# praateekmahajan/moving-mnist-vae

Hardware: AMD Instinct MI355X
Metric: frames/sec/GPU VAE train step, 20×64×64 batch; ELBO vs CPU ref (higher is better)
Workload: dtype bf16; 1 GPU; BASELINE configs[1]: 256 clips x 20 frames x 64x64 per GPU per step (=5120 frames), conv-VAE z=128, Gaussian NLL sigma=0.1 + KL (normal_vae_1_kl_0_mmd), Adam, random-init weights, Bernoulli(0.0521) q=2 labels; parallelism=dp1, rccl_ranks=1, grad_exchange=none, bn=per-rank batch statistics

## Files before the change

### include/mmvae.h

```cpp
#ifndef MMVAE_H_
#define MMVAE_H_

#include <stddef.h>
#include <stdint.h>

#ifdef __cplusplus
extern "C" {
#endif

#if defined(__GNUC__)
#define MMVAE_API __attribute__((visibility("default")))
#else
#define MMVAE_API
#endif

#define MMVAE_OK 0
#define MMVAE_ERR_ARG (-1)
#define MMVAE_ERR_HIP (-2)
#define MMVAE_ERR_WORKSPACE (-3)
#define MMVAE_ERR_UNSUPPORTED (-4)

#define MMVAE_F32 0
#define MMVAE_BF16 1
#define MMVAE_FP8 2
// ... 189 lines not shown
                               const float* b2, const void* ys, const float* ss, const float* bs, float* partials, float* wpartials,
                               int N, int H, int W, void* stream);
MMVAE_API int mmvae_tail_join_bwd_apply(int dtype, const float* d_raw, const float* weight, int out_planes, const void* y2, const float* s2,
                              const float* b2, const void* ys, const float* ss, const float* bs, const float* A2, const float* B2,
                              const float* C2, const float* As, const float* Bs, const float* Cs, void* dy2, void* dys, int N, int H, int W,
                              void* stream);
MMVAE_API int mmvae_upblock_bwd_fused(const float* d_raw, const float* tail_weight, const void* y2, const float* s2, const float* b2,
                            const void* ys, const float* ss, const float* bs, const float* A2, const float* B2, const float* C2,
                            const float* As, const float* Bs, const float* Cs, const void* y1, const float* s1, const float* b1,
                            const float* w_conv2, float* dw_conv2, void* d_a1, float* bn1_sums, const void* xin, const float* sx,
                            const float* bx, const float* w_up, float* dw_up, void* g_in, int N, void* scratch, void* stream);
MMVAE_API int mmvae_upblock_tail_fwd(const void* y1, const float* s1, const float* b1, const float* w2, const void* x_in, const float* sx,
                                     const float* bx, const float* wu, const float* s2, const float* b2, const float* ss, const float* bs,
                                     const float* tail_weight, const float* tail_bias, float* r_raw, float* stats, int N, void* scratch,
                                     void* stream);
MMVAE_API int mmvae_join_conv1x1_fwd(const void* y2, const float* s2, const float* b2, const void* ys, const float* ss, const float* bs,
                           const float* w_conv1, int C, void* out, void* y1, float* stats, int64_t npix, void* scratch, void* stream);
MMVAE_API int mmvae_conv1x1_bwd_fused(const void* d_a1, const void* y1, const float* s1, const float* b1, const float* A1, const float* B1,
                            const float* C1, const void* xin, const float* sx, const float* bx, const float* w_conv1, float* dw_conv1,
                            void* g_in, int64_t rows, void* scratch, void* stream);
typedef struct mmvae_pixelcnn mmvae_pixelcnn;
MMVAE_API int mmvae_pixelcnn_create(mmvae_pixelcnn** out, int in_channels, int intermediate_channels, int out_channels, int layers, int dtype);
MMVAE_API void mmvae_pixelcnn_destroy(mmvae_pixelcnn* net);
MMVAE_API int64_t mmvae_pixelcnn_num_params(mmvae_pixelcnn* net);
MMVAE_API size_t mmvae_pixelcnn_workspace_bytes(mmvae_pixelcnn* net, int N, int S);
MMVAE_API int mmvae_pixelcnn_fwd(mmvae_pixelcnn* net, int N, int S, const float* x, const float* params, void* workspace, size_t workspace_bytes,
                       float* out, void* stream);
MMVAE_API int mmvae_pixelcnn_bwd(mmvae_pixelcnn* net, int N, int S, const float* x, const float* d_out, const float* params, float* grads,
                       void* workspace, size_t workspace_bytes, float* d_x, void* stream);
MMVAE_API size_t mmvae_pixelcnn_sample_workspace_bytes(mmvae_pixelcnn* net, int N, int S);
// ... 11 lines not shown
```

### moving-mnist-vae_amd/_lib.py

```python
from __future__ import annotations

import ctypes
import os
from ctypes import POINTER, c_char_p, c_double, c_float, c_int, c_int32, c_int64, c_size_t, c_uint64, c_void_p

import torch

_HERE = os.path.dirname(os.path.abspath(__file__))
LIB_PATH = os.environ.get("MMVAE_LIB_PATH") or os.path.join(_HERE, "libmmvae_hip.so")
_lib = None
ABI_VERSION = 3
SUM_PARTIALS = 1025
BN_SCRATCH_BYTES = 16 << 20
STEM_SCRATCH_BYTES = 12800

P = c_void_p

PROTOTYPES = {
    "mmvae_abi_version": (c_int, []),
    "mmvae_last_error": (c_char_p, []),
    "mmvae_net_create": (c_int, [POINTER(c_void_p), c_int, c_int, c_int, c_int, c_int, c_int]),
    "mmvae_net_create_ex": (c_int, [POINTER(c_void_p), c_int, c_int, c_int, c_int, c_int, c_int, c_int]),
    "mmvae_net_destroy": (None, [P]),
    "mmvae_net_sizes": (c_int, [P, POINTER(c_int64), POINTER(c_int64), POINTER(c_int32), POINTER(c_int64), POINTER(c_int32)]),
# ... 68 lines not shown
    "mmvae_net_set_sync_bn_comm": (c_int, [P, P]),
    "mmvae_net_set_sync_bn_comm2": (c_int, [P, P, P]),
    "mmvae_convT_bwd_fused": (c_int, [c_int, P, P, P, P, P, c_int, c_int, c_int, c_int, c_int, c_int, c_int, c_int, P, P, c_int, P, P, P, P, P, P]),
    "mmvae_batchnorm_fwd": (c_int, [c_int, P, c_int64, c_int, P, P, P, P, P, c_float, c_float, c_int, P, P, P, P, P]),
    "mmvae_batchnorm_bwd": (c_int, [c_int, P, P, P, c_int64, c_int, P, P, P, P, P, P, P, P]),
    "mmvae_stem_fwd": (c_int, [c_int, P, P, P, c_int, c_int, P, P, P]),
    "mmvae_stem_bwd": (c_int, [c_int, P, P, P, P, P, P, P, P, P, P, P, P, c_int, c_int, P, P]),
    "mmvae_tail_join_fwd": (c_int, [c_int, P, P, P, P, P, P, P, P, P, P, c_int, c_int, c_int, P]),
    "mmvae_tail_join_fwd_stream": (c_int, [c_int, P, P, P, P, P, P, P, P, P, P, c_int, c_int, c_int, P]),
    "mmvae_tail_join_bwd_reduce": (c_int, [c_int, P, P, c_int, P, P, P, P, P, P, P, P, c_int, c_int, c_int, P]),
    "mmvae_tail_join_bwd_apply": (c_int, [c_int, P, P, c_int, P, P, P, P, P, P, P, P, P, P, P, P, P, P, c_int, c_int, c_int, P]),
    "mmvae_upblock_bwd_fused": (c_int, [P] * 27 + [c_int, P, P]),
    "mmvae_join_conv1x1_fwd": (c_int, [P, P, P, P, P, P, P, c_int, P, P, P, c_int64, P, P]),
    "mmvae_conv1x1_bwd_fused": (c_int, [P] * 13 + [c_int64, P, P]),
    "mmvae_upblock_tail_fwd": (c_int, [P] * 16 + [c_int, P, P]),
    "mmvae_pixelcnn_create": (c_int, [POINTER(c_void_p), c_int, c_int, c_int, c_int, c_int]),
    "mmvae_pixelcnn_destroy": (None, [P]),
    "mmvae_pixelcnn_num_params": (c_int64, [P]),
    "mmvae_pixelcnn_workspace_bytes": (c_size_t, [P, c_int, c_int]),
    "mmvae_pixelcnn_fwd": (c_int, [P, c_int, c_int, P, P, P, c_size_t, P, P]),
    "mmvae_pixelcnn_bwd": (c_int, [P, c_int, c_int, P, P, P, P, P, c_size_t, P, P]),
    "mmvae_pixelcnn_sample_workspace_bytes": (c_size_t, [P, c_int, c_int]),
    "mmvae_pixelcnn_sample": (c_int, [P, c_int, c_int, P, c_int, P, c_int, P, c_float, c_float, P, P, c_size_t, P, P, P, P]),
    "mmvae_convert": (c_int, [c_int, c_int, P, P, c_int64, P]),
}


class MmvaeError(RuntimeError):
    pass

# ... 71 lines not shown
```

### moving-mnist-vae_amd/csrc/capi.cpp

```cpp
#include <cstring>
#include <new>

#include "../../include/mmvae.h"
#include "conv_ops.hpp"
#include "pixel_net.hpp"
#include "quantiser_fit.hpp"
#include "resample.hpp"
#include "vae_net.hpp"

namespace mmvae { const char* last_error(); }
using namespace mmvae;

struct mmvae_net { Net* net; };
struct mmvae_comm { Comm* c; };

static inline hipStream_t stream_of(void* s) { return static_cast<hipStream_t>(s); }

extern "C" {

int mmvae_abi_version(void) { return MMVAE_ABI_VERSION; }
const char* mmvae_last_error(void) { return last_error(); }

int mmvae_net_create(mmvae_net** out, int in_channels, int z, int out_channels, int image_size, int need_logvar, int dtype) {
  return mmvae_net_create_ex(out, in_channels, z, out_channels, image_size, need_logvar, dtype, 1);
// ... 592 lines not shown
  }
  return launch_partial_rowsum(L.bn_part, nb, 32, bn1_sums, stream_of(st));
}
int mmvae_upblock_tail_fwd(const void* y1, const float* s1, const float* b1, const float* w2, const void* xin, const float* sx, const float* bx,
                           const float* wu, const float* s2, const float* b2, const float* ss, const float* bs, const float* tw, const float* bias,
                           float* r_raw, float* stats, int N, void* scratch, void* st) {
  if (!scratch || !y1 || !s1 || !b1 || !w2 || !xin || !wu || !s2 || !b2 || !ss || !bs || !tw || !r_raw || N < 1 || ((sx != nullptr) != (bx != nullptr))) {
    set_error("upblock_tail_fwd: bad argument"); return MMVAE_ERR_ARG;
  }
  char* sc = static_cast<char*>(scratch);
  const ConvGeom g = geom_for(1, 16, 16, 4, 2, 1);
  int rc = op_pack_up(DT_BF16, g, w2, sc, stream_of(st)); if (rc < 0) return rc;
  rc = op_pack_up(DT_BF16, g, wu, sc + 8192, stream_of(st)); if (rc < 0) return rc;
  return launch_up5_tail_fwd(y1, s1, b1, sc, xin, sx, bx, sc + 8192, s2, b2, ss, bs, tw, bias, r_raw, stats, N, stream_of(st));
}
int mmvae_conv1x1_bwd_fused(const void* da1, const void* y1, const float* s1, const float* b1, const float* A1, const float* B1, const float* C1,
                            const void* xin, const float* sx, const float* bx, const float* w1, float* dw1, void* gin, int64_t rows, void* scratch,
                            void* st) {
  if (!scratch || !da1 || !y1 || !s1 || !b1 || !A1 || !B1 || !C1 || !xin || !w1 || !dw1 || !gin || rows < 1 || ((sx != nullptr) != (bx != nullptr))) {
    set_error("conv1x1_bwd_fused: bad argument"); return MMVAE_ERR_ARG;
  }
  char* sc = static_cast<char*>(scratch);
  const ConvGeom g = geom_for(0, 16, 16, 1, 1, 0);
  int rc = op_pack_up(DT_BF16, g, w1, sc, stream_of(st)); if (rc < 0) return rc;
  Conv1BwdLaunch C;
  C.da1 = da1; C.y1 = y1; C.ms = s1; C.mb = b1; C.A = A1; C.B = B1; C.C = C1; C.xin = xin; C.pxs = sx; C.pxb = bx; C.w1u = sc; C.gin = gin;
  C.part = reinterpret_cast<float*>(sc + 4096); C.nrows = (long)rows;
  const int nb = launch_conv1_bwd_stream(C, stream_of(st));
  if (nb < 0) return nb;
  WgradReduceArgs u; std::memset(&u, 0, sizeof(u));
// ... 15 lines not shown
```

### moving-mnist-vae_amd/csrc/conv_fstream.hip

```cpp
#include <hip/hip_runtime.h>

#include <stdlib.h>
#include <string.h>

#include "kernels.hpp"
#include "tile_common.hpp"

namespace mmvae {

struct Conv3StreamArgs {
  const void* x; const void* w; const void* wsc; void* y; void* ysc;
  const float* pro_scale; const float* pro_shift; int pro_relu;
  float* stats; float* stats_sc;
  const void* ym; const float* ms; const float* mb;
  int N, Ho, Hi;
  int HS, nunits;
};

template <int S, bool SC, bool PRO, bool BS = false>
__global__ __launch_bounds__(256, 2) void conv3_stream_kernel(Conv3StreamArgs a) {
  static_assert(!BS || (S == 1 && !SC && !PRO), "backward sums: the stride-1 data gradient");
  constexpr int KS = 3, PAD = 1, WO = 16, WI = S * WO, CB = 64;
  constexpr int WL = WI + 2;
  constexpr int ROWB = WL * CB;
// ... 331 lines not shown
  }
  st1 = row16_sum(st1); st2 = row16_sum(st2);
  float* sb = reinterpret_cast<float*>(smem);
  if (lane == 0) { sb[wv * 2] = st1; sb[wv * 2 + 1] = st2; }
  __syncthreads();
  if (a.stats && t < 2) a.stats[(long)blockIdx.x * 2 + t] = (sb[t] + sb[2 + t]) + (sb[4 + t] + sb[6 + t]);
}

struct ConvT4StreamArgs {
  const void* x; const void* w; void* y;
  const float* pro_scale; const float* pro_shift; int pro_relu;
  float* stats;
  int N, Hi, HS, nunits;
};

template <int WIN, bool PRO, bool F8O = false>
__global__ __launch_bounds__(256, 3) void convT4_stream_kernel(ConvT4StreamArgs a) {
  constexpr int CB = 32, WL = WIN + 2, ROWB = WL * CB, NSLOT = 4, NPRIME = 2;
  constexpr int CBO = F8O ? 16 : 32;
  constexpr int OROWB = 2 * WIN * CBO;
  constexpr int WAVE_LDS = NSLOT * ROWB + OROWB;
  constexpr int XV = (WIN * CB + 1023) / 1024;
  constexpr int NPT = WIN / 16;
  extern __shared__ __attribute__((aligned(16))) char smem[];
  const int t = threadIdx.x, lane = t & 63, wv = __builtin_amdgcn_readfirstlane(t >> 6), gq = lane >> 4, r = lane & 15;
  char* ring = smem + 1024 + wv * WAVE_LDS;
  char* orow = ring + NSLOT * ROWB;
  for (int s = 0; s < NSLOT; ++s) {
    if (lane < 2) *reinterpret_cast<Vec16*>(ring + s * ROWB + lane * 16) = Vec16{{0, 0, 0, 0}};
    else if (lane < 4) *reinterpret_cast<Vec16*>(ring + s * ROWB + (WL - 1) * CB + (lane - 2) * 16) = Vec16{{0, 0, 0, 0}};
  }
  Vec16 wA[4][2];
#pragma unroll
  for (int p = 0; p < 4; ++p)
#pragma unroll
    for (int th = 0; th < 2; ++th)
// ... 26 lines not shown
  };
  auto commit = [&](int u, int q) {
    const int n = u / nstrips, q0 = (u - n * nstrips) * a.HS;
    const int row = q0 + q - NPRIME + 1;
    if (xlane) {
      Vec16 v = xv;
      if (PRO && row >= 0 && row < a.Hi) {
        float f[8];
        Elem<bf16_t>::unpack(v, f);
#pragma unroll
        for (int j = 0; j < 8; ++j) f[j] = fmaxf(f[j] * psc[j] + psh[j], lo);
        v = Elem<bf16_t>::pack(f);
      }
      *reinterpret_cast<Vec16*>(ring + ((row + 4 * NSLOT) % NSLOT) * ROWB + CB + lane * 16) = v;
    }
    (void)n; (void)XV;
  };
  int u = u_first, q = 0;
  if (u < u_end) issue(u, 0);
  while (u < u_end) {
    commit(u, q);
    int un = u, qn = q + 1;
    if (qn == nq) { un = u + u_step; qn = 0; }
    if (un < u_end) issue(un, qn);
    __builtin_amdgcn_sched_barrier(0);
    if (q >= NPRIME) {
      const int n = u / nstrips, iq = (u - n * nstrips) * a.HS + q - NPRIME;
#pragma unroll
      for (int ph = 0; ph < 2; ++ph) {
#pragma unroll
        for (int pw = 0; pw < 2; ++pw) {
// ... 2 lines not shown
          for (int pt = 0; pt < NPT; ++pt) acc[pt] = (f32x4){0, 0, 0, 0};
#pragma unroll
          for (int th = 0; th < 2; ++th) {
            const int dh = ph == 0 ? (th == 0 ? 0 : -1) : (th == 0 ? 1 : 0);
            const char* rowp = ring + ((iq + dh + 4 * NSLOT) % NSLOT) * ROWB;
#pragma unroll
            for (int pt = 0; pt < NPT; ++pt) {
              const Vec16 b = *reinterpret_cast<const Vec16*>(rowp + (16 * pt + r + dwl[pw] + 1) * CB + (gq & 1) * 16);
              acc[pt] = mma_bf16(wA[2 * ph + pw][th], b, acc[pt]);
            }
          }
#pragma unroll
          for (int pt = 0; pt < NPT; ++pt) {
#pragma unroll
            for (int j = 0; j < 4; ++j) { st1[j] += acc[pt][j]; st2[j] += acc[pt][j] * acc[pt][j]; }
            if constexpr (F8O) {
              *reinterpret_cast<uint32_t*>(orow + (2 * (16 * pt + r) + pw) * CBO + gq * 4) = pack4_fp8(acc[pt][0], acc[pt][1], acc[pt][2], acc[pt][3]);
            } else {
              uint2 o;
              o.x = pack2_bf16(acc[pt][0], acc[pt][1]); o.y = pack2_bf16(acc[pt][2], acc[pt][3]);
              *reinterpret_cast<uint2*>(orow + (2 * (16 * pt + r) + pw) * CB + gq * 8) = o;
            }
          }
        }
        asm volatile("" ::: "memory");
        char* dst = reinterpret_cast<char*>(a.y) + (((long)n * (2 * a.Hi) + 2 * iq + ph) * (2 * WIN)) * CBO;
#pragma unroll
        for (int k = 0; k < OROWB / 1024; ++k) *reinterpret_cast<Vec16*>(dst + (lane + 64 * k) * 16) = *reinterpret_cast<const Vec16*>(orow + (lane + 64 * k) * 16);
      }
    }
    __builtin_amdgcn_sched_barrier(0);
    u = un; q = qn;
  }
  float* sb = reinterpret_cast<float*>(smem);
#pragma unroll
  for (int j = 0; j < 4; ++j) {
    const float v1 = row16_sum(st1[j]), v2 = row16_sum(st2[j]);
    if (r == 0) { sb[wv * 32 + 4 * gq + j] = v1; sb[wv * 32 + 16 + 4 * gq + j] = v2; }
  }
  __syncthreads();
  if (a.stats && t < 32) a.stats[(long)blockIdx.x * 32 + t] = (sb[t] + sb[32 + t]) + (sb[64 + t] + sb[96 + t]);
}

struct Up5TailFwdArgs {
  const void* y1; const float* p1s; const float* p1b; const void* w2;
  const void* xin; const float* pxs; const float* pxb; const void* wu;
  const float* s2; const float* b2; const float* ss; const float* bs;
  const float* w; const float* bias; float* r_raw; float* stats;
  int N, HS, nunits;
};

template <bool PRO_X>
__global__ __launch_bounds__(256, 2) void up5_tail_fwd_kernel(Up5TailFwdArgs a) {
  constexpr int WIN = 32, Hi = 32, W = 64, H = 64, CB = 32;
  constexpr int IWL = WIN + 2, IROWB = IWL * CB, NSLOT = 4;
  constexpr int JWL = W + 2, JROWB = JWL * CB;
  constexpr int WAVE_LDS = 2 * NSLOT * IROWB + NSLOT * JROWB;
  extern __shared__ __attribute__((aligned(16))) char smem[];
  const int t = threadIdx.x, lane = t & 63, wv = __builtin_amdgcn_readfirstlane(t >> 6), gq = lane >> 4, r = lane & 15;
  char* ringA = smem + 64 + wv * WAVE_LDS;
  char* ringX = ringA + NSLOT * IROWB;
  char* ringJ = ringX + NSLOT * IROWB;
  for (int sl = 0; sl < NSLOT; ++sl) {
    if (lane < 2) { *reinterpret_cast<Vec16*>(ringA + sl * IROWB + lane * 16) = Vec16{{0, 0, 0, 0}}; *reinterpret_cast<Vec16*>(ringX + sl * IROWB + lane * 16) = Vec16{{0, 0, 0, 0}}; }
    else if (lane < 4) { *reinterpret_cast<Vec16*>(ringA + sl * IROWB + (IWL - 1) * CB + (lane - 2) * 16) = Vec16{{0, 0, 0, 0}}; *reinterpret_cast<Vec16*>(ringX + sl * IROWB + (IWL - 1) * CB + (lane - 2) * 16) = Vec16{{0, 0, 0, 0}}; }
    else if (lane < 6) *reinterpret_cast<Vec16*>(ringJ + sl * JROWB + (lane - 4) * 16) = Vec16{{0, 0, 0, 0}};
    else if (lane < 8) *reinterpret_cast<Vec16*>(ringJ + sl * JROWB + (JWL - 1) * CB + (lane - 6) * 16) = Vec16{{0, 0, 0, 0}};
// ... 72 lines not shown
    *reinterpret_cast<Vec16*>(ringX + slot * IROWB + CB + lane * 16) = cx;
    (void)n;
  };
  int u = u_first, q = 0;
  if (u < u_end) issue(u, 0);
  while (u < u_end) {
    commit(u, q);
    int un = u, qn = q + 1;
    if (qn == nq) { un = u + u_step; qn = 0; }
    if (un < u_end) issue(un, qn);
    __builtin_amdgcn_sched_barrier(0);
    if (q >= NPRIME) {
      const int n = u / nstrips, q0 = (u - n * nstrips) * a.HS;
      const int iq = q0 - 1 + q - NPRIME;
      const bool inside = iq >= 0 && iq < Hi;
#pragma unroll
      for (int ph = 0; ph < 2; ++ph) {
        char* jrow = ringJ + ((2 * iq + ph + 8 * NSLOT) % NSLOT) * JROWB;
        if (!inside) {
          for (int i = lane; i < (W * CB) / 16; i += 64) *reinterpret_cast<Vec16*>(jrow + CB + i * 16) = Vec16{{0, 0, 0, 0}};
          continue;
        }
#pragma unroll
        for (int pw = 0; pw < 2; ++pw) {
          f32x4 acc2[2], accS[2];
#pragma unroll
          for (int pt = 0; pt < 2; ++pt) { acc2[pt] = (f32x4){0, 0, 0, 0}; accS[pt] = (f32x4){0, 0, 0, 0}; }
#pragma unroll
          for (int th = 0; th < 2; ++th) {
            const int dh = ph == 0 ? (th == 0 ? 0 : -1) : (th == 0 ? 1 : 0);
            const int sl = (iq + dh + 4 * NSLOT) % NSLOT;
#pragma unroll
            for (int pt = 0; pt < 2; ++pt) {
              const int off = sl * IROWB + (16 * pt + r + dwl[pw] + 1) * CB + (gq & 1) * 16;
              acc2[pt] = mma_bf16(w2A[2 * ph + pw][th], *reinterpret_cast<const Vec16*>(ringA + off), acc2[pt]);
              accS[pt] = mma_bf16(wuA[2 * ph + pw][th], *reinterpret_cast<const Vec16*>(ringX + off), accS[pt]);
            }
          }
#pragma unroll
          for (int pt = 0; pt < 2; ++pt) {
            float o[4];
#pragma unroll
            for (int j = 0; j < 4; ++j) o[j] = fmaxf(acc2[pt][j] * js2[j] + jb[j] + accS[pt][j] * jss[j], 0.f);
            *reinterpret_cast<uint2*>(jrow + (1 + 2 * (16 * pt + r) + pw) * CB + gq * 8) = make_uint2(pack2_bf16(o[0], o[1]), pack2_bf16(o[2], o[3]));
          }
        }
      }
      asm volatile("" ::: "memory");
#pragma unroll
      for (int k = 0; k < 2; ++k) {
        const int oh = 2 * iq - 1 + k;
        if (oh < 2 * q0 || oh >= 2 * (q0 + a.HS) || oh < 0 || oh >= H) continue;
        f32x4 acc[4];
        const char* row01 = ringJ + ((oh - 1 + (gq >> 1) + 8 * NSLOT) % NSLOT) * JROWB;
        const char* row2 = ringJ + ((oh + 1 + 8 * NSLOT) % NSLOT) * JROWB;
#pragma unroll
        for (int pt = 0; pt < 4; ++pt) {
          const int po = (16 * pt + r + 1) * CB + (gq & 1) * 16;
          acc[pt] = mma_bf16(wT[0], *reinterpret_cast<const Vec16*>(row01 + po), (f32x4){0, 0, 0, 0});
// ... 33 lines not shown
    __builtin_amdgcn_sched_barrier(0);
    u = un; q = qn;
  }
  st1 = row16_sum(st1); st2 = row16_sum(st2);
  float* sb = reinterpret_cast<float*>(smem);
  if (lane == 0) { sb[wv * 2] = st1; sb[wv * 2 + 1] = st2; }
  __syncthreads();
  if (a.stats && t < 2) a.stats[(long)blockIdx.x * 2 + t] = (sb[t] + sb[2 + t]) + (sb[4 + t] + sb[6 + t]);
}

bool up5_tail_fwd_ok(int dt, int OC, int C, int Cin, int Hin, int Hout) {
  return dt == DT_BF16 && OC == 1 && C == 16 && Cin == 16 && Hin == 32 && Hout == 64;
}
int launch_up5_tail_fwd(const void* y1, const float* p1s, const float* p1b, const void* w2_up, const void* xin, const float* pxs, const float* pxb,
                        const void* wu_up, const float* s2, const float* b2, const float* ss, const float* bs, const float* w, const float* bias,
                        float* r_raw, float* stats, int N, hipStream_t s) {
  Up5TailFwdArgs a; memset(&a, 0, sizeof(a));
  a.y1 = y1; a.p1s = p1s; a.p1b = p1b; a.w2 = w2_up; a.xin = xin; a.pxs = pxs; a.pxb = pxb; a.wu = wu_up;
  a.s2 = s2; a.b2 = b2; a.ss = ss; a.bs = bs; a.w = w; a.bias = bias; a.r_raw = r_raw; a.stats = stats;
  a.N = N; a.HS = 16; a.nunits = N * (32 / a.HS);
  int gx = 512;
  while (gx > 1 && (long)gx * 4 > a.nunits) gx -= gx > 8 ? 8 : 1;
  const size_t lds = 64 + 4 * (size_t)(2 * 4 * 34 * 32 + 4 * 66 * 32);
  static bool attr_set = false;
  if (!attr_set) {
    hipError_t e = hipFuncSetAttribute(reinterpret_cast<const void*>(&up5_tail_fwd_kernel<false>), hipFuncAttributeMaxDynamicSharedMemorySize, 160 * 1024);
    if (e == hipSuccess) e = hipFuncSetAttribute(reinterpret_cast<const void*>(&up5_tail_fwd_kernel<true>), hipFuncAttributeMaxDynamicSharedMemorySize, 160 * 1024);
    if (e != hipSuccess) { set_error("up5_tail_fwd: hipFuncSetAttribute: %s", hipGetErrorString(e)); return MMVAE_ERR_HIP; }
    attr_set = true;
  }
  if (pxs) hipLaunchKernelGGL(up5_tail_fwd_kernel<true>, dim3(gx), dim3(256), lds, s, a);
  else hipLaunchKernelGGL(up5_tail_fwd_kernel<false>, dim3(gx), dim3(256), lds, s, a);
  note_launch_bytes((double)N * (2.0 * 32 * 32 * 16 * 2 + 64 * 64 * 4.0));
  const int rc = check_launch("up5_tail_fwd");
  return rc ? rc : gx;
}

bool convT4_stream_ok(int dt, int Cin, int Cout, int k, int s, int p, int Hin, int Win) {
  return dt == DT_BF16 && Cin == 16 && Cout == 16 && k == 4 && s == 2 && p == 1 && Hin == Win && (Win == 32 || Win == 16);
}
int launch_convT4_stream(int dt, const void* x, const void* w_up, void* y, const float* pro_scale, const float* pro_shift, int pro_relu, float* stats,
                         int N, int Hin, hipStream_t s, int f8out) {
  if (!convT4_stream_ok(dt, 16, 16, 4, 2, 1, Hin, Hin)) { set_error("convT4_stream: bf16, 16 -> 16 channels, k4 s2 p1, 16x16 or 32x32 input"); return MMVAE_ERR_UNSUPPORTED; }
  ConvT4StreamArgs a; memset(&a, 0, sizeof(a));
  a.x = x; a.w = w_up; a.y = y; a.pro_scale = pro_scale; a.pro_shift = pro_shift; a.pro_relu = pro_relu; a.stats = stats;
  a.N = N; a.Hi = Hin; a.HS = Hin % 8 == 0 ? 8 : Hin; a.nunits = N * (Hin / a.HS);
  int gx = Hin == 32 ? 1024 : 768;
  while (gx > 8 && (long)gx * 4 > a.nunits) gx -= 8;
  const bool pro = pro_scale != nullptr;
  const size_t lds = 1024 + 4 * (size_t)(4 * (Hin + 2) * 32 + 2 * Hin * 32);
  if (f8out && Hin != 32) { set_error("convT4_stream: e4m3 output only for the 32x32 -> 64x64 layers"); return MMVAE_ERR_UNSUPPORTED; }
  if (f8out) { if (pro) hipLaunchKernelGGL((convT4_stream_kernel<32, true, true>), dim3(gx), dim3(256), lds, s, a); else hipLaunchKernelGGL((convT4_stream_kernel<32, false, true>), dim3(gx), dim3(256), lds, s, a); }
  else if (Hin == 32) { if (pro) hipLaunchKernelGGL((convT4_stream_kernel<32, true>), dim3(gx), dim3(256), lds, s, a); else hipLaunchKernelGGL((convT4_stream_kernel<32, false>), dim3(gx), dim3(256), lds, s, a); }
  else { if (pro) hipLaunchKernelGGL((convT4_stream_kernel<16, true>), dim3(gx), dim3(256), lds, s, a); else hipLaunchKernelGGL((convT4_stream_kernel<16, false>), dim3(gx), dim3(256), lds, s, a); }
  note_launch_bytes((double)N * 16 * (2.0 + (f8out ? 4.0 : 8.0)) * Hin * Hin);
  const int rc = check_launch("convT4_stream");
  return rc ? rc : gx;
}

bool tail_fwd_stream_ok(int dt, int OC, int H, int W) {
  return dt == DT_BF16 && OC == 1 && W == 64 && H == 64;
}
int launch_tail_fwd_stream(int dt, const void* y2, const float* s2, const float* b2, const void* ys, const float* ss, const float* bs, const float* w,
                           const float* bias, float* r_raw, float* stats, int N, int H, int W, hipStream_t s, int f8in) {
  if (!tail_fwd_stream_ok(dt, 1, H, W)) { set_error("tail_fwd_stream: bf16, one output plane, 64x64"); return MMVAE_ERR_UNSUPPORTED; }
  TailFwdStreamArgs a; memset(&a, 0, sizeof(a));
  a.y2 = y2; a.ys = ys; a.s2 = s2; a.b2 = b2; a.ss = ss; a.bs = bs; a.w = w; a.bias = bias; a.r_raw = r_raw; a.stats = stats;
  a.N = N; a.H = H; a.HS = 16; a.nunits = N * (H / a.HS);
  int gx = 768;
  while (gx > 1 && (long)gx * 4 > a.nunits) gx -= gx > 8 ? 8 : 1;
// ... 10 lines not shown
```

### moving-mnist-vae_amd/csrc/kernels.hpp

```cpp
#pragma once
#include "common.hpp"

namespace mmvae {

enum DType : int { DT_F32 = 0, DT_BF16 = 1 };
inline size_t dtype_size(int dt) { return dt == DT_F32 ? 4 : 2; }

struct Tap { int dh, dw; };
constexpr int kMaxTaps = 25;
constexpr int kMaxPhases = 4;
struct Phase { int ph, pw, Hq, Wq, ntaps, tap0; long w_off;  };
struct GatherArgs {
  const void* x; const void* w; void* y;
  const float* pro_scale; const float* pro_shift; int pro_relu;
  const float* bias;
  float* stats;
  int accumulate;
  int N, Hi, Wi, Cin, Ho, Wo, Cout;
  int SI, SO;
  int nphase; Phase phases[kMaxPhases]; Tap taps[kMaxTaps];
  int cin_vecs;
  int x_planar, x_planes;
  int y_planes;
  const void* x2; const void* w2; int Cin2, x2_ph, x2_pw;
// ... 139 lines not shown
bool stem_bwd_fusable(int S);
bool conv3_stream_ok(int dt, int Cin, int Cout, int k, int s, int p, int Hin, int Win);
int launch_conv3_stream_bwd(int dt, const void* dy, const void* w_flipped, void* dx, const void* ym, const float* ms, const float* mb, float* sums,
                            int N, int H, hipStream_t s);
int launch_conv3_stream(int dt, int stride, const void* x, const void* w, const void* wsc, void* y, void* ysc, const float* pro_scale,
                        const float* pro_shift, int pro_relu, float* stats, float* stats_sc, int N, int Ho, hipStream_t s);
bool convT4_stream_ok(int dt, int Cin, int Cout, int k, int s, int p, int Hin, int Win);
int launch_convT4_stream(int dt, const void* x, const void* w_up, void* y, const float* pro_scale, const float* pro_shift, int pro_relu, float* stats,
                         int N, int Hin, hipStream_t s, int f8out = 0);
bool tail_fwd_stream_ok(int dt, int OC, int H, int W);
int launch_tail_fwd_stream(int dt, const void* y2, const float* s2, const float* b2, const void* ys, const float* ss, const float* bs, const float* w,
                           const float* bias, float* r_raw, float* stats, int N, int H, int W, hipStream_t s, int f8in = 0);
bool up5_tail_fwd_ok(int dt, int OC, int C, int Cin, int Hin, int Hout);
int launch_up5_tail_fwd(const void* y1, const float* p1s, const float* p1b, const void* w2_up, const void* xin, const float* pxs, const float* pxb,
                        const void* wu_up, const float* s2, const float* b2, const float* ss, const float* bs, const float* w, const float* bias,
                        float* r_raw, float* stats, int N, hipStream_t s);
bool stem_fwd_stream_ok(int dt, int S);
int launch_stem_fwd_stream(int dt, const void* x, const float* w, void* y, float* stats, int N, int S, hipStream_t s);
int stem_bwd_part_floats();
int launch_stem_gram(int dt, const void* x, float* scratch, long scratch_cap_floats, double* R, int N, int S, int Ho, int Wo, hipStream_t s);
int launch_stem_bwd(int dt, const void* g, const void* y0, const void* x, const float* ms, const float* mb, float* partials,
                    long partials_cap_floats, int N, int S, int Ho, int Wo, hipStream_t s);
bool stem_bwd_dg_ok(int dt, int S);
int launch_stem_bwd_dg(const void* dy1, const void* dys, const void* wd1, const void* wds, const void* y0, const void* x, const float* ms, const float* mb,
                       float* partials, long partials_cap_floats, int N, int S, int Ho, int Wo, hipStream_t s);
int launch_stem_bwd_finalize(const float* partials, int nparts, const double* R, const float* w, const float* global_sums, double count,
                             const float* gamma, const float* mean, const float* istd, float* dgamma, float* dbeta, float* dW, hipStream_t s);

int launch_chan_stats_nhwc(int dt, const void* y, long npix, int C, float* partials, hipStream_t s);
int chan_stats_parts(long npix, int C);
struct BnFinalizeArgs {
// ... 132 lines not shown
```

### moving-mnist-vae_amd/csrc/vae_net.cpp

```cpp
#include "vae_net.hpp"

#include <algorithm>
#include <cmath>
#include <cstdlib>
#include <cstring>

#include "conv_ops.hpp"

namespace mmvae {

#define MM_TRY(expr)            \
  do {                          \
    int rc__ = (expr);          \
    if (rc__ < 0) return rc__;  \
  } while (0)

static inline long align_up(long v, long a) { return (v + a - 1) / a * a; }
static inline int down_size(int H, int k, int s, int p) { return conv_down_size(H, k, s, p); }

void Net::add_entry(const std::string& name, std::initializer_list<int> shape, int kind, long off) {
  Entry e; e.name = name; e.ndim = (int)shape.size(); e.kind = kind; e.offset = off;
  int i = 0; for (int d : shape) e.shape[i++] = d;
  for (; i < 4; ++i) e.shape[i] = 1;
  entries.push_back(e);
// ... 723 lines not shown
  if (!training) MM_TRY(fold_bn_eval(ps, 1, s));
  MM_TRY(launch_convert(DT_F32, dt(), encv, base + P.enc_t, (long)N * cfg.z, s));
  int np = run_up(ps, dstem, base + P.enc_t, 1, 1, base + P.y0d, 2, 2, nullptr, nullptr, 0, stats, 0, s);
  MM_TRY(np);
  MM_TRY(bn_fwd(ps, dbn0, np, (double)N * 4, s, 0, dstem.wscale));
  const void* xin = base + P.y0d;
  const float* xs = ps.rows(dbn0).scale;
  const float* xb = ps.rows(dbn0).shift;
  const int nd = (int)dec.size();
  if (cfg.blocks > 1) {
    MM_TRY(fill_consts(ps, s));
    MM_TRY(launch_affine_act(dt(), base + P.y0d, xs, xb, 1, base + P.act0d, (long)N * 4, 128, s));
    xin = base + P.act0d; xs = xb = nullptr;
  }
  int c1_done = 0;
  for (int i = 0; i < nd; ++i) {
    Block& B = dec[i];
    const double cnt = (double)N * B.Hout * B.Wout;
    const BnRows r1 = ps.rows(B.b1), r2 = ps.rows(B.b2);
    const Shortcut sc = ps.shortcut(B, xin);
    if (!B.identity) {
      MM_TRY(side_fork(s));
      hipStream_t ss = wgrad_stream(s);
      if (!B.cs.fp8 && convT4_stream_ok(dt(), B.cs.D0, B.cs.D1, B.cs.k, B.cs.s, B.cs.p, B.Hin, B.Win))
        np = launch_convT4_stream(dt(), xin, ps.packed(B.cs.packU), base + B.ys, xs, xb, 1, stats ? stats + kPartialFloats : nullptr,
                                  N, B.Hin, ss, (store8 && i == nd - 1) ? 1 : 0);
      else
        np = run_up(ps, B.cs, xin, B.Hin, B.Win, base + B.ys, B.Hout, B.Wout, xs, xb, 1, stats ? stats + kPartialFloats : nullptr, 0, ss);
      MM_TRY(np);
      MM_TRY(bn_fwd(ps, B.bs, np, cnt, ss, kPartialFloats, B.cs.wscale));
    }
    np = c1_done > 0 ? c1_done : run_down(ps, B.c1, xin, B.Hin, B.Win, base + B.y1, B.Hin, B.Win, xs, xb, 1, stats, 0, dt(), s);
    c1_done = 0;
    MM_TRY(np);
    MM_TRY(bn_fwd(ps, B.b1, np, (double)N * B.Hin * B.Win, s, 0, B.c1.wscale));
    if (B.identity)
      np = run_down(ps, B.c2, base + B.y1, B.Hin, B.Win, base + B.y2, B.Hout, B.Wout, r1.scale, r1.shift, 1, stats, 0, dt(), s);
    else
      if (!B.c2.fp8 && convT4_stream_ok(dt(), B.c2.D0, B.c2.D1, B.c2.k, B.c2.s, B.c2.p, B.Hin, B.Win))
        np = launch_convT4_stream(dt(), base + B.y1, ps.packed(B.c2.packU), base + B.y2, r1.scale, r1.shift, 1, stats, N, B.Hin, s,
                                  (store8 && i == nd - 1) ? 1 : 0);
      else
        np = run_up(ps, B.c2, base + B.y1, B.Hin, B.Win, base + B.y2, B.Hout, B.Wout, r1.scale, r1.shift, 1, stats, 0, s);
    MM_TRY(np);
    MM_TRY(bn_fwd(ps, B.b2, np, cnt, s, 0, B.c2.wscale));
    if (!B.identity) MM_TRY(side_join(s));
    if (i == nd - 1 && tail_fwd_fused()) break;
    if (i == nd - 1 && store8) { set_error("fp8 storage of the last up-block needs the fused tail kernels"); return MMVAE_ERR_UNSUPPORTED; }
    const bool fuse_c1 = i + 1 < nd && !B.identity && !dec[i + 1].identity && !dec[i + 1].c1.fp8 && dec[i + 1].c1.k == 1 && dec[i + 1].c1.s == 1 &&
                         dec[i + 1].c1.D1 == B.C && !dec[i + 1].c1.fragD && dec[i + 1].c1.wscale == 1.f &&
                         join_conv1_fwd_ok(dt(), B.C, dec[i + 1].c1.D0, (long)N * B.Hout * B.Wout);
    if (fuse_c1) {
      c1_done = launch_join_conv1_fwd(B.C, base + B.y2, r2.scale, r2.shift, sc.y, sc.scale, sc.shift, ps.packed(dec[i + 1].c1.packD),
                                      base + B.out, base + dec[i + 1].y1, stats, (long)N * B.Hout * B.Wout, s);
      MM_TRY(c1_done);
    } else
    MM_TRY(launch_join_fwd(dt(), base + B.y2, r2.scale, r2.shift, sc.y, sc.scale, sc.shift, base + B.out,
                           (long)N * B.Hout * B.Wout, B.C, s));
    xin = base + B.out; xs = xb = nullptr;
  }
  float* r_raw = reinterpret_cast<float*>(base + P.r_raw);
  if (tail_fwd_fused()) {
    const Block& B = dec.back();
    const BnRows r1 = ps.rows(B.b1), r2 = ps.rows(B.b2);
    const Shortcut sc = ps.shortcut(B, xin);
    if (!store8 && !B.identity && !B.c2.fp8 && !B.cs.fp8 && tail_fwd_stream_ok(dt(), cfg.out_ch, Sd, Sd) &&
        up5_tail_fwd_ok(dt(), cfg.out_ch, B.C, B.Cin, B.Hin, B.Hout) && convT4_stream_ok(dt(), B.c2.D0, B.c2.D1, B.c2.k, B.c2.s, B.c2.p, B.Hin, B.Win))
      np = launch_up5_tail_fwd(base + B.y1, r1.scale, r1.shift, ps.packed(B.c2.packU), xin, xs, xb, ps.packed(B.cs.packU), r2.scale, r2.shift,
                               sc.scale, sc.shift, params + tail.off, params + tail_bias, r_raw, stats, N, s);
    else if (tail_fwd_stream_ok(dt(), cfg.out_ch, Sd, Sd))
      np = launch_tail_fwd_stream(dt(), base + B.y2, r2.scale, r2.shift, sc.y, sc.scale, sc.shift, params + tail.off, params + tail_bias,
                                  r_raw, stats, N, Sd, Sd, s, store8 ? 1 : 0);
    else if (store8) { set_error("fp8 storage of the last up-block needs tail_fwd_stream"); return MMVAE_ERR_UNSUPPORTED; }
    else
      np = launch_tail_join_fwd(dt(), base + B.y2, r2.scale, r2.shift, sc.y, sc.scale, sc.shift, params + tail.off, params + tail_bias,
                                r_raw, stats, N, Sd, Sd, s);
  } else {
    GatherArgs a; std::memset(&a, 0, sizeof(a));
    a.x = xin; a.w = ps.packed(tail_pack_f); a.y = r_raw; a.bias = params + tail_bias; a.stats = stats; a.y_planes = cfg.out_ch;
    a.N = N; a.Hi = Sd; a.Wi = Sd; a.Cin = 16; a.Ho = Sd; a.Wo = Sd; a.Cout = 16; a.SI = 1; a.SO = 1;
    a.nphase = 1; a.phases[0] = Phase{0, 0, Sd, Sd, 9, 0, 0};
    for (int kh = 0; kh < 3; ++kh) for (int kw = 0; kw < 3; ++kw) a.taps[kh * 3 + kw] = Tap{kh - 1, kw - 1};
    np = launch_gather_gemm(dt(), DT_F32, a, s);
  }
// ... 203 lines not shown
```

Measured before the change: 855,300 frames/s.

## Make last up-block convT passes statistics-only and store outputs from fused tail kernel

On the fused up5 tail route, the last decoder block's two transposed convolutions (main and shortcut) now run in a statistics-only mode that computes BN sums without writing y2/ys. The fused tail kernel, which recomputes these convolutions anyway, writes the pre-BN y2 and ys outputs itself through permlane swaps when a training step needs them. In inference mode without stats the convT launches are skipped entirely. This removes one full write of two 64x64x16 bf16 tensors per frame, at the cost of extra stores and registers in the tail kernel.

```diff
diff --git a/include/mmvae.h b/include/mmvae.h
--- a/include/mmvae.h
+++ b/include/mmvae.h
@@ -227,6 +227,12 @@
                                      const float* bx, const float* wu, const float* s2, const float* b2, const float* ss, const float* bs,
                                      const float* tail_weight, const float* tail_bias, float* r_raw, float* stats, int N, void* scratch,
                                      void* stream);
+MMVAE_API int mmvae_upblock_tail_fwd_store(const void* y1, const float* s1, const float* b1, const float* w2, const void* x_in, const float* sx,
+                                           const float* bx, const float* wu, const float* s2, const float* b2, const float* ss, const float* bs,
+                                           const float* tail_weight, const float* tail_bias, float* r_raw, float* stats, void* y2, void* ys,
+                                           int N, void* scratch, void* stream);
+MMVAE_API int mmvae_convT4_stats(int dtype, const void* x, const float* weight, const float* pro_scale, const float* pro_shift, float* stats,
+                                 int N, int e4m3_out, void* scratch, void* stream);
 MMVAE_API int mmvae_join_conv1x1_fwd(const void* y2, const float* s2, const float* b2, const void* ys, const float* ss, const float* bs,
                            const float* w_conv1, int C, void* out, void* y1, float* stats, int64_t npix, void* scratch, void* stream);
 MMVAE_API int mmvae_conv1x1_bwd_fused(const void* d_a1, const void* y1, const float* s1, const float* b1, const float* A1, const float* B1,
diff --git a/moving-mnist-vae_amd/_lib.py b/moving-mnist-vae_amd/_lib.py
--- a/moving-mnist-vae_amd/_lib.py
+++ b/moving-mnist-vae_amd/_lib.py
@@ -106,6 +106,8 @@
     "mmvae_join_conv1x1_fwd": (c_int, [P, P, P, P, P, P, P, c_int, P, P, P, c_int64, P, P]),
     "mmvae_conv1x1_bwd_fused": (c_int, [P] * 13 + [c_int64, P, P]),
     "mmvae_upblock_tail_fwd": (c_int, [P] * 16 + [c_int, P, P]),
+    "mmvae_upblock_tail_fwd_store": (c_int, [P] * 18 + [c_int, P, P]),
+    "mmvae_convT4_stats": (c_int, [c_int, P, P, P, P, P, c_int, c_int, P, P]),
     "mmvae_pixelcnn_create": (c_int, [POINTER(c_void_p), c_int, c_int, c_int, c_int, c_int]),
     "mmvae_pixelcnn_destroy": (None, [P]),
     "mmvae_pixelcnn_num_params": (c_int64, [P]),
diff --git a/moving-mnist-vae_amd/csrc/capi.cpp b/moving-mnist-vae_amd/csrc/capi.cpp
--- a/moving-mnist-vae_amd/csrc/capi.cpp
+++ b/moving-mnist-vae_amd/csrc/capi.cpp
@@ -630,6 +630,27 @@
   rc = op_pack_up(DT_BF16, g, wu, sc + 8192, stream_of(st)); if (rc < 0) return rc;
   return launch_up5_tail_fwd(y1, s1, b1, sc, xin, sx, bx, sc + 8192, s2, b2, ss, bs, tw, bias, r_raw, stats, N, stream_of(st));
 }
+int mmvae_upblock_tail_fwd_store(const void* y1, const float* s1, const float* b1, const float* w2, const void* xin, const float* sx, const float* bx,
+                                 const float* wu, const float* s2, const float* b2, const float* ss, const float* bs, const float* tw,
+                                 const float* bias, float* r_raw, float* stats, void* y2, void* ys, int N, void* scratch, void* st) {
+  if (!scratch || !y1 || !s1 || !b1 || !w2 || !xin || !wu || !s2 || !b2 || !ss || !bs || !tw || !r_raw || !y2 || !ys || N < 1 ||
+      ((sx != nullptr) != (bx != nullptr))) {
+    set_error("upblock_tail_fwd_store: bad argument"); return MMVAE_ERR_ARG;
+  }
+  char* sc = static_cast<char*>(scratch);
+  const ConvGeom g = geom_for(1, 16, 16, 4, 2, 1);
+  int rc = op_pack_up(DT_BF16, g, w2, sc, stream_of(st)); if (rc < 0) return rc;
+  rc = op_pack_up(DT_BF16, g, wu, sc + 8192, stream_of(st)); if (rc < 0) return rc;
+  return launch_up5_tail_fwd(y1, s1, b1, sc, xin, sx, bx, sc + 8192, s2, b2, ss, bs, tw, bias, r_raw, stats, N, stream_of(st), y2, ys);
+}
+int mmvae_convT4_stats(int dt, const void* x, const float* w, const float* ps, const float* pb, float* stats, int N, int e4m3_out, void* scratch,
+                       void* st) {
+  if (!scratch || !x || !w || !stats || N < 1 || ((ps != nullptr) != (pb != nullptr))) { set_error("convT4_stats: bad argument"); return MMVAE_ERR_ARG; }
+  if (dt != DT_BF16) { set_error("convT4_stats: bf16 only"); return MMVAE_ERR_UNSUPPORTED; }
+  if (e4m3_out) { set_error("convT4_stats: the e4m3 storage mode has no statistics-only form"); return MMVAE_ERR_UNSUPPORTED; }
+  int rc = op_pack_up(dt, geom_for(1, 16, 16, 4, 2, 1), w, scratch, stream_of(st)); if (rc < 0) return rc;
+  return launch_convT4_stream(dt, x, scratch, nullptr, ps, pb, 1, stats, N, 32, stream_of(st));
+}
 int mmvae_conv1x1_bwd_fused(const void* da1, const void* y1, const float* s1, const float* b1, const float* A1, const float* B1, const float* C1,
                             const void* xin, const float* sx, const float* bx, const float* w1, float* dw1, void* gin, int64_t rows, void* scratch,
                             void* st) {
diff --git a/moving-mnist-vae_amd/csrc/conv_fstream.hip b/moving-mnist-vae_amd/csrc/conv_fstream.hip
--- a/moving-mnist-vae_amd/csrc/conv_fstream.hip
+++ b/moving-mnist-vae_amd/csrc/conv_fstream.hip
@@ -369,12 +369,13 @@
   int N, Hi, HS, nunits;
 };
 
-template <int WIN, bool PRO, bool F8O = false>
+template <int WIN, bool PRO, bool F8O = false, bool NOY = false>
 __global__ __launch_bounds__(256, 3) void convT4_stream_kernel(ConvT4StreamArgs a) {
+  static_assert(!NOY || !F8O, "statistics-only: the bf16 forms");
   constexpr int CB = 32, WL = WIN + 2, ROWB = WL * CB, NSLOT = 4, NPRIME = 2;
   constexpr int CBO = F8O ? 16 : 32;
   constexpr int OROWB = 2 * WIN * CBO;
-  constexpr int WAVE_LDS = NSLOT * ROWB + OROWB;
+  constexpr int WAVE_LDS = NSLOT * ROWB + (NOY ? 0 : OROWB);
   constexpr int XV = (WIN * CB + 1023) / 1024;
   constexpr int NPT = WIN / 16;
   extern __shared__ __attribute__((aligned(16))) char smem[];
@@ -431,7 +432,7 @@
       }
       *reinterpret_cast<Vec16*>(ring + ((row + 4 * NSLOT) % NSLOT) * ROWB + CB + lane * 16) = v;
     }
-    (void)n; (void)XV;
+    (void)n; (void)XV; (void)orow;
   };
   int u = u_first, q = 0;
   if (u < u_end) issue(u, 0);
@@ -464,7 +465,8 @@
           for (int pt = 0; pt < NPT; ++pt) {
 #pragma unroll
             for (int j = 0; j < 4; ++j) { st1[j] += acc[pt][j]; st2[j] += acc[pt][j] * acc[pt][j]; }
-            if constexpr (F8O) {
+            if constexpr (NOY) {
+            } else if constexpr (F8O) {
               *reinterpret_cast<uint32_t*>(orow + (2 * (16 * pt + r) + pw) * CBO + gq * 4) = pack4_fp8(acc[pt][0], acc[pt][1], acc[pt][2], acc[pt][3]);
             } else {
               uint2 o;
@@ -473,11 +475,14 @@
             }
           }
         }
-        asm volatile("" ::: "memory");
-        char* dst = reinterpret_cast<char*>(a.y) + (((long)n * (2 * a.Hi) + 2 * iq + ph) * (2 * WIN)) * CBO;
-#pragma unroll
-        for (int k = 0; k < OROWB / 1024; ++k) *reinterpret_cast<Vec16*>(dst + (lane + 64 * k) * 16) = *reinterpret_cast<const Vec16*>(orow + (lane + 64 * k) * 16);
-      }
+        if constexpr (!NOY) {
+          asm volatile("" ::: "memory");
+          char* dst = reinterpret_cast<char*>(a.y) + (((long)n * (2 * a.Hi) + 2 * iq + ph) * (2 * WIN)) * CBO;
+#pragma unroll
+          for (int k = 0; k < OROWB / 1024; ++k) *reinterpret_cast<Vec16*>(dst + (lane + 64 * k) * 16) = *reinterpret_cast<const Vec16*>(orow + (lane + 64 * k) * 16);
+        }
+      }
+      (void)n;
     }
     __builtin_amdgcn_sched_barrier(0);
     u = un; q = qn;
@@ -497,10 +502,11 @@
   const void* xin; const float* pxs; const float* pxb; const void* wu;
   const float* s2; const float* b2; const float* ss; const float* bs;
   const float* w; const float* bias; float* r_raw; float* stats;
+  void* y2; void* ys;
   int N, HS, nunits;
 };
 
-template <bool PRO_X>
+template <bool PRO_X, bool STORE = false>
 __global__ __launch_bounds__(256, 2) void up5_tail_fwd_kernel(Up5TailFwdArgs a) {
   constexpr int WIN = 32, Hi = 32, W = 64, H = 64, CB = 32;
   constexpr int IWL = WIN + 2, IROWB = IWL * CB, NSLOT = 4;
@@ -603,6 +609,7 @@
       const int n = u / nstrips, q0 = (u - n * nstrips) * a.HS;
       const int iq = q0 - 1 + q - NPRIME;
       const bool inside = iq >= 0 && iq < Hi;
+      const bool own = STORE && iq >= q0 && iq < q0 + a.HS;
 #pragma unroll
       for (int ph = 0; ph < 2; ++ph) {
         char* jrow = ringJ + ((2 * iq + ph + 8 * NSLOT) % NSLOT) * JROWB;
@@ -610,6 +617,8 @@
           for (int i = lane; i < (W * CB) / 16; i += 64) *reinterpret_cast<Vec16*>(jrow + CB + i * 16) = Vec16{{0, 0, 0, 0}};
           continue;
         }
+        uint2 k2[2][2], ks[2][2];
+        (void)k2; (void)ks; (void)own;
 #pragma unroll
         for (int pw = 0; pw < 2; ++pw) {
           f32x4 acc2[2], accS[2];
@@ -632,6 +641,25 @@
 #pragma unroll
             for (int j = 0; j < 4; ++j) o[j] = fmaxf(acc2[pt][j] * js2[j] + jb[j] + accS[pt][j] * jss[j], 0.f);
             *reinterpret_cast<uint2*>(jrow + (1 + 2 * (16 * pt + r) + pw) * CB + gq * 8) = make_uint2(pack2_bf16(o[0], o[1]), pack2_bf16(o[2], o[3]));
+            if constexpr (STORE) {
+              k2[pw][pt] = make_uint2(pack2_bf16(acc2[pt][0], acc2[pt][1]), pack2_bf16(acc2[pt][2], acc2[pt][3]));
+              ks[pw][pt] = make_uint2(pack2_bf16(accS[pt][0], accS[pt][1]), pack2_bf16(accS[pt][2], accS[pt][3]));
+            }
+          }
+        }
+        if constexpr (STORE) {
+          if (own) {
+            char* const o2 = reinterpret_cast<char*>(a.y2) + (((long)n * H + 2 * iq + ph) * W) * CB + (gq & 1) * CB + (gq >> 1) * 16;
+            char* const oS = reinterpret_cast<char*>(a.ys) + (o2 - reinterpret_cast<char*>(a.y2));
+#pragma unroll
+            for (int pt = 0; pt < 2; ++pt) {
+              const auto x2 = __builtin_amdgcn_permlane16_swap(k2[0][pt].x, k2[1][pt].x, false, false);
+              const auto y2 = __builtin_amdgcn_permlane16_swap(k2[0][pt].y, k2[1][pt].y, false, false);
+              const auto xS = __builtin_amdgcn_permlane16_swap(ks[0][pt].x, ks[1][pt].x, false, false);
+              const auto yS = __builtin_amdgcn_permlane16_swap(ks[0][pt].y, ks[1][pt].y, false, false);
+              *reinterpret_cast<Vec16*>(o2 + 2 * (16 * pt + r) * CB) = Vec16{{x2[0], y2[0], x2[1], y2[1]}};
+              *reinterpret_cast<Vec16*>(oS + 2 * (16 * pt + r) * CB) = Vec16{{xS[0], yS[0], xS[1], yS[1]}};
+            }
           }
         }
       }
@@ -695,10 +723,12 @@
 }
 int launch_up5_tail_fwd(const void* y1, const float* p1s, const float* p1b, const void* w2_up, const void* xin, const float* pxs, const float* pxb,
                         const void* wu_up, const float* s2, const float* b2, const float* ss, const float* bs, const float* w, const float* bias,
-                        float* r_raw, float* stats, int N, hipStream_t s) {
+                        float* r_raw, float* stats, int N, hipStream_t s, void* y2, void* ys) {
+  if ((y2 != nullptr) != (ys != nullptr)) { set_error("up5_tail_fwd: y2 and ys go together"); return MMVAE_ERR_ARG; }
+  const bool store = y2 != nullptr;
   Up5TailFwdArgs a; memset(&a, 0, sizeof(a));
   a.y1 = y1; a.p1s = p1s; a.p1b = p1b; a.w2 = w2_up; a.xin = xin; a.pxs = pxs; a.pxb = pxb; a.wu = wu_up;
-  a.s2 = s2; a.b2 = b2; a.ss = ss; a.bs = bs; a.w = w; a.bias = bias; a.r_raw = r_raw; a.stats = stats;
+  a.s2 = s2; a.b2 = b2; a.ss = ss; a.bs = bs; a.w = w; a.bias = bias; a.r_raw = r_raw; a.stats = stats; a.y2 = y2; a.ys = ys;
   a.N = N; a.HS = 16; a.nunits = N * (32 / a.HS);
   int gx = 512;
   while (gx > 1 && (long)gx * 4 > a.nunits) gx -= gx > 8 ? 8 : 1;
@@ -707,12 +737,17 @@
   if (!attr_set) {
     hipError_t e = hipFuncSetAttribute(reinterpret_cast<const void*>(&up5_tail_fwd_kernel<false>), hipFuncAttributeMaxDynamicSharedMemorySize, 160 * 1024);
     if (e == hipSuccess) e = hipFuncSetAttribute(reinterpret_cast<const void*>(&up5_tail_fwd_kernel<true>), hipFuncAttributeMaxDynamicSharedMemorySize, 160 * 1024);
+    if (e == hipSuccess) e = hipFuncSetAttribute(reinterpret_cast<const void*>(&up5_tail_fwd_kernel<false, true>), hipFuncAttributeMaxDynamicSharedMemorySize, 160 * 1024);
+    if (e == hipSuccess) e = hipFuncSetAttribute(reinterpret_cast<const void*>(&up5_tail_fwd_kernel<true, true>), hipFuncAttributeMaxDynamicSharedMemorySize, 160 * 1024);
     if (e != hipSuccess) { set_error("up5_tail_fwd: hipFuncSetAttribute: %s", hipGetErrorString(e)); return MMVAE_ERR_HIP; }
     attr_set = true;
   }
-  if (pxs) hipLaunchKernelGGL(up5_tail_fwd_kernel<true>, dim3(gx), dim3(256), lds, s, a);
+  if (store) {
+    if (pxs) hipLaunchKernelGGL((up5_tail_fwd_kernel<true, true>), dim3(gx), dim3(256), lds, s, a);
+    else hipLaunchKernelGGL((up5_tail_fwd_kernel<false, true>), dim3(gx), dim3(256), lds, s, a);
+  } else if (pxs) hipLaunchKernelGGL(up5_tail_fwd_kernel<true>, dim3(gx), dim3(256), lds, s, a);
   else hipLaunchKernelGGL(up5_tail_fwd_kernel<false>, dim3(gx), dim3(256), lds, s, a);
-  note_launch_bytes((double)N * (2.0 * 32 * 32 * 16 * 2 + 64 * 64 * 4.0));
+  note_launch_bytes((double)N * (2.0 * 32 * 32 * 16 * 2 + 64 * 64 * 4.0 + (store ? 2.0 * 64 * 64 * 16 * 2 : 0.0)));
   const int rc = check_launch("up5_tail_fwd");
   return rc ? rc : gx;
 }
@@ -729,12 +764,17 @@
   int gx = Hin == 32 ? 1024 : 768;
   while (gx > 8 && (long)gx * 4 > a.nunits) gx -= 8;
   const bool pro = pro_scale != nullptr;
-  const size_t lds = 1024 + 4 * (size_t)(4 * (Hin + 2) * 32 + 2 * Hin * 32);
+  const bool noy = y == nullptr;
+  const size_t lds = 1024 + 4 * (size_t)(4 * (Hin + 2) * 32 + (noy ? 0 : 2 * Hin * 32));
   if (f8out && Hin != 32) { set_error("convT4_stream: e4m3 output only for the 32x32 -> 64x64 layers"); return MMVAE_ERR_UNSUPPORTED; }
-  if (f8out) { if (pro) hipLaunchKernelGGL((convT4_stream_kernel<32, true, true>), dim3(gx), dim3(256), lds, s, a); else hipLaunchKernelGGL((convT4_stream_kernel<32, false, true>), dim3(gx), dim3(256), lds, s, a); }
+  if (noy && f8out) { set_error("convT4_stream: the statistics-only form (y == NULL) has no e4m3 variant"); return MMVAE_ERR_UNSUPPORTED; }
+  if (noy && !stats) { set_error("convT4_stream: y == NULL needs stats"); return MMVAE_ERR_ARG; }
+  if (noy && Hin == 32) { if (pro) hipLaunchKernelGGL((convT4_stream_kernel<32, true, false, true>), dim3(gx), dim3(256), lds, s, a); else hipLaunchKernelGGL((convT4_stream_kernel<32, false, false, true>), dim3(gx), dim3(256), lds, s, a); }
+  else if (noy) { if (pro) hipLaunchKernelGGL((convT4_stream_kernel<16, true, false, true>), dim3(gx), dim3(256), lds, s, a); else hipLaunchKernelGGL((convT4_stream_kernel<16, false, false, true>), dim3(gx), dim3(256), lds, s, a); }
+  else if (f8out) { if (pro) hipLaunchKernelGGL((convT4_stream_kernel<32, true, true>), dim3(gx), dim3(256), lds, s, a); else hipLaunchKernelGGL((convT4_stream_kernel<32, false, true>), dim3(gx), dim3(256), lds, s, a); }
   else if (Hin == 32) { if (pro) hipLaunchKernelGGL((convT4_stream_kernel<32, true>), dim3(gx), dim3(256), lds, s, a); else hipLaunchKernelGGL((convT4_stream_kernel<32, false>), dim3(gx), dim3(256), lds, s, a); }
   else { if (pro) hipLaunchKernelGGL((convT4_stream_kernel<16, true>), dim3(gx), dim3(256), lds, s, a); else hipLaunchKernelGGL((convT4_stream_kernel<16, false>), dim3(gx), dim3(256), lds, s, a); }
-  note_launch_bytes((double)N * 16 * (2.0 + (f8out ? 4.0 : 8.0)) * Hin * Hin);
+  note_launch_bytes((double)N * 16 * (2.0 + (noy ? 0.0 : f8out ? 4.0 : 8.0)) * Hin * Hin);
   const int rc = check_launch("convT4_stream");
   return rc ? rc : gx;
 }
diff --git a/moving-mnist-vae_amd/csrc/kernels.hpp b/moving-mnist-vae_amd/csrc/kernels.hpp
--- a/moving-mnist-vae_amd/csrc/kernels.hpp
+++ b/moving-mnist-vae_amd/csrc/kernels.hpp
@@ -177,7 +177,7 @@
 bool up5_tail_fwd_ok(int dt, int OC, int C, int Cin, int Hin, int Hout);
 int launch_up5_tail_fwd(const void* y1, const float* p1s, const float* p1b, const void* w2_up, const void* xin, const float* pxs, const float* pxb,
                         const void* wu_up, const float* s2, const float* b2, const float* ss, const float* bs, const float* w, const float* bias,
-                        float* r_raw, float* stats, int N, hipStream_t s);
+                        float* r_raw, float* stats, int N, hipStream_t s, void* y2 = nullptr, void* ys = nullptr);
 bool stem_fwd_stream_ok(int dt, int S);
 int launch_stem_fwd_stream(int dt, const void* x, const float* w, void* y, float* stats, int N, int S, hipStream_t s);
 int stem_bwd_part_floats();
diff --git a/moving-mnist-vae_amd/csrc/vae_net.cpp b/moving-mnist-vae_amd/csrc/vae_net.cpp
--- a/moving-mnist-vae_amd/csrc/vae_net.cpp
+++ b/moving-mnist-vae_amd/csrc/vae_net.cpp
@@ -761,16 +761,25 @@
     xin = base + P.act0d; xs = xb = nullptr;
   }
   int c1_done = 0;
+  bool up5_route = false;
+  if (nd > 0 && tail_fwd_fused()) {
+    const Block& B = dec.back();
+    up5_route = !store8 && !B.identity && !B.c2.fp8 && !B.cs.fp8 && tail_fwd_stream_ok(dt(), cfg.out_ch, Sd, Sd) &&
+                up5_tail_fwd_ok(dt(), cfg.out_ch, B.C, B.Cin, B.Hin, B.Hout) && convT4_stream_ok(dt(), B.c2.D0, B.c2.D1, B.c2.k, B.c2.s, B.c2.p, B.Hin, B.Win) &&
+                convT4_stream_ok(dt(), B.cs.D0, B.cs.D1, B.cs.k, B.cs.s, B.cs.p, B.Hin, B.Win);
+  }
   for (int i = 0; i < nd; ++i) {
     Block& B = dec[i];
     const double cnt = (double)N * B.Hout * B.Wout;
     const BnRows r1 = ps.rows(B.b1), r2 = ps.rows(B.b2);
     const Shortcut sc = ps.shortcut(B, xin);
+    const bool stats_only = up5_route && i == nd - 1;
     if (!B.identity) {
       MM_TRY(side_fork(s));
       hipStream_t ss = wgrad_stream(s);
-      if (!B.cs.fp8 && convT4_stream_ok(dt(), B.cs.D0, B.cs.D1, B.cs.k, B.cs.s, B.cs.p, B.Hin, B.Win))
-        np = launch_convT4_stream(dt(), xin, ps.packed(B.cs.packU), base + B.ys, xs, xb, 1, stats ? stats + kPartialFloats : nullptr,
+      if (stats_only && !stats) np = 1;
+      else if (!B.cs.fp8 && convT4_stream_ok(dt(), B.cs.D0, B.cs.D1, B.cs.k, B.cs.s, B.cs.p, B.Hin, B.Win))
+        np = launch_convT4_stream(dt(), xin, ps.packed(B.cs.packU), stats_only ? nullptr : base + B.ys, xs, xb, 1, stats ? stats + kPartialFloats : nullptr,
                                   N, B.Hin, ss, (store8 && i == nd - 1) ? 1 : 0);
       else
         np = run_up(ps, B.cs, xin, B.Hin, B.Win, base + B.ys, B.Hout, B.Wout, xs, xb, 1, stats ? stats + kPartialFloats : nullptr, 0, ss);
@@ -784,8 +793,9 @@
     if (B.identity)
       np = run_down(ps, B.c2, base + B.y1, B.Hin, B.Win, base + B.y2, B.Hout, B.Wout, r1.scale, r1.shift, 1, stats, 0, dt(), s);
     else
-      if (!B.c2.fp8 && convT4_stream_ok(dt(), B.c2.D0, B.c2.D1, B.c2.k, B.c2.s, B.c2.p, B.Hin, B.Win))
-        np = launch_convT4_stream(dt(), base + B.y1, ps.packed(B.c2.packU), base + B.y2, r1.scale, r1.shift, 1, stats, N, B.Hin, s,
+      if (stats_only && !stats) np = 1;
+      else if (!B.c2.fp8 && convT4_stream_ok(dt(), B.c2.D0, B.c2.D1, B.c2.k, B.c2.s, B.c2.p, B.Hin, B.Win))
+        np = launch_convT4_stream(dt(), base + B.y1, ps.packed(B.c2.packU), stats_only ? nullptr : base + B.y2, r1.scale, r1.shift, 1, stats, N, B.Hin, s,
                                   (store8 && i == nd - 1) ? 1 : 0);
       else
         np = run_up(ps, B.c2, base + B.y1, B.Hin, B.Win, base + B.y2, B.Hout, B.Wout, r1.scale, r1.shift, 1, stats, 0, s);
@@ -811,10 +821,10 @@
     const Block& B = dec.back();
     const BnRows r1 = ps.rows(B.b1), r2 = ps.rows(B.b2);
     const Shortcut sc = ps.shortcut(B, xin);
-    if (!store8 && !B.identity && !B.c2.fp8 && !B.cs.fp8 && tail_fwd_stream_ok(dt(), cfg.out_ch, Sd, Sd) &&
-        up5_tail_fwd_ok(dt(), cfg.out_ch, B.C, B.Cin, B.Hin, B.Hout) && convT4_stream_ok(dt(), B.c2.D0, B.c2.D1, B.c2.k, B.c2.s, B.c2.p, B.Hin, B.Win))
+    if (up5_route)
       np = launch_up5_tail_fwd(base + B.y1, r1.scale, r1.shift, ps.packed(B.c2.packU), xin, xs, xb, ps.packed(B.cs.packU), r2.scale, r2.shift,
-                               sc.scale, sc.shift, params + tail.off, params + tail_bias, r_raw, stats, N, s);
+                               sc.scale, sc.shift, params + tail.off, params + tail_bias, r_raw, stats, N, s,
+                               stats ? base + B.y2 : nullptr, stats ? base + B.ys : nullptr);
     else if (tail_fwd_stream_ok(dt(), cfg.out_ch, Sd, Sd))
       np = launch_tail_fwd_stream(dt(), base + B.y2, r2.scale, r2.shift, sc.y, sc.scale, sc.shift, params + tail.off, params + tail_bias,
                                   r_raw, stats, N, Sd, Sd, s, store8 ? 1 : 0);
```

New measurement: 866,800 frames/s, median of 6. 1.01x the previous value.
